# springmeyer/cov-tiles

Measured on AMD Instinct MI355X. Metric: GB/s raw COVT bytes decoded + Mvertices/s, z2–z14 tile batch, 1/2/4/8 GPU, higher is better.
Workload: dtype int32

## Files before the change

### cov-tiles_amd/csrc/covt_decode.hip

```cpp
#include <hip/hip_runtime.h>
#include <stdint.h>

#include "covt.h"
#include "covt_internal.h"
#include "covt_wave.h"
#include "covt_walk.h"

namespace covt {

constexpr int kWin = 1024;
constexpr int kFpfBlock = 256;
constexpr int kFpfPage = 65536;
constexpr int kFpfBcCap = 3 * kFpfPage / kFpfBlock + kFpfPage;

#ifndef COVT_LONG_STREAM
#define COVT_LONG_STREAM 16384
#endif
#ifndef COVT_LONG_PRIO
#define COVT_LONG_PRIO 2
#endif
#ifndef COVT_RLE_SHORT_SPAN
#define COVT_RLE_SHORT_SPAN 448
#endif
#ifndef COVT_CHUNK_PRIO
// ... 211 lines not shown
    const int32_t steps = (int32_t)wave_max((uint32_t)((nch + 15) >> 4));
    for (int32_t c0 = 0; c0 < 16 * steps; c0 += 16) {
        const int32_t ch = c0 + q;
        if (ch < nch) {
            const int32_t i = head + K * ch;
            int4 w;
            if (E == 8) {
                const int64_t v0 = val(i), v1 = val(i + 1);
                w = make_int4((int)v0, (int)(v0 >> 32), (int)v1, (int)(v1 >> 32));
            } else {
                w = make_int4((int)val(i), (int)val(i + 1), (int)val(i + 2), (int)val(i + 3));
            }
            st_out16((int32_t*)(arr + (int64_t)(o + i) * E), w);
        }
    }
}

template <int OP, int K>
__device__ __forceinline__ void sink_values(const uint32_t (&vin)[K], int64_t base, int32_t first, int32_t count,
                                            int nb, uint8_t* __restrict__ out, Carry& c) {
    const int l = lane_id();
    const bool full = first == 0 && count >= 64 * K;
    const int32_t s0 = l * K - first;
    const bool lfull = full || (s0 >= 0 && s0 + K <= count);
    const int64_t i0 = base + (int64_t)l * K;
    bool ok[K];
    uint32_t v[K];
#pragma unroll
    for (int k = 0; k < K; ++k) {
        ok[k] = full || (s0 + k >= 0 && s0 + k < count);
        v[k] = ok[k] ? vin[k] : 0u;
    }
    auto st32 = [&](const int32_t (&r)[K]) {
        int32_t* o = (int32_t*)out + i0;
        if (K == 4 && lfull) {
            st_out16(o, make_int4(r[0], r[K > 1 ? 1 : 0], r[K > 2 ? 2 : 0], r[K > 3 ? 3 : 0]));
        } else {
#pragma unroll
            for (int k = 0; k < K; ++k)
                if (ok[k]) st_out(o + k, r[k]);
        }
    };
    auto st64 = [&](const int64_t (&r)[K]) {
        int64_t* o = (int64_t*)out + i0;
#pragma unroll
        for (int k = 0; k < K; ++k)
            if (ok[k]) st_out(o + k, r[k]);
    };
    if constexpr (OP == COVT_OP_VARINT_I32 || OP == COVT_OP_VARINT_ZZ_I32) {
        int32_t r[K];
#pragma unroll
        for (int k = 0; k < K; ++k) r[k] = OP == COVT_OP_VARINT_I32 ? (int32_t)v[k] : zz32(v[k]);
        st32(r);
    } else if constexpr (OP == COVT_OP_VARINT_I32_AS_I64 || OP == COVT_OP_VARINT_ZZ_I32_AS_I64) {
        int64_t r[K];
#pragma unroll
        for (int k = 0; k < K; ++k) r[k] = OP == COVT_OP_VARINT_I32_AS_I64 ? (int64_t)(int32_t)v[k] : (int64_t)zz32(v[k]);
        st64(r);
    } else if constexpr (OP == COVT_OP_VARINT_ZZ_DELTA_I32 || OP == COVT_OP_FPF_ZZ_DELTA_I32 ||
                         OP == COVT_OP_VARINT_ZZ_DELTA_I64) {
        uint32_t sacc[K];
        uint32_t acc = 0;
#pragma unroll
        for (int k = 0; k < K; ++k) {
            acc += (uint32_t)zz32(v[k]);
            sacc[k] = acc;
        }
        const uint32_t inc = incl_scan(acc);
        const uint32_t pre = c.x + inc - acc;
        if constexpr (OP == COVT_OP_VARINT_ZZ_DELTA_I64) {
            int64_t r[K];
#pragma unroll
            for (int k = 0; k < K; ++k) r[k] = (int64_t)(int32_t)(pre + sacc[k]);
            st64(r);
        } else {
            int32_t r[K];
#pragma unroll
            for (int k = 0; k < K; ++k) r[k] = (int32_t)(pre + sacc[k]);
            st32(r);
        }
        c.x += lane_bcast(inc, 63);
    } else if constexpr (OP == COVT_OP_VARINT_ZZ_DELTA_XY || OP == COVT_OP_FPF_ZZ_DELTA_XY) {
        uint32_t sx[K], sy[K];
        uint32_t ax = 0, ay = 0;
        const uint32_t par0 = (uint32_t)(i0 & 1);
#pragma unroll
        for (int k = 0; k < K; ++k) {
            const uint32_t z = (uint32_t)zz32(v[k]);
            const bool isx = ((par0 + k) & 1u) == 0;
            ax += isx ? z : 0u;
            ay += isx ? 0u : z;
            sx[k] = ax;
            sy[k] = ay;
        }
        const uint32_t incx = incl_scan(ax), incy = incl_scan(ay);
        const uint32_t prex = c.x + incx - ax, prey = c.y + incy - ay;
        int32_t r[K];
#pragma unroll
        for (int k = 0; k < K; ++k) r[k] = (int32_t)((((par0 + k) & 1u) == 0) ? (prex + sx[k]) : (prey + sy[k]));
        st32(r);
        c.x += lane_bcast(incx, 63);
        c.y += lane_bcast(incy, 63);
    } else if constexpr (OP == COVT_OP_VARINT_DELTA_MORTON || OP == COVT_OP_FPF_DELTA_MORTON) {
        uint32_t sacc[K];
        uint32_t acc = 0;
#pragma unroll
        for (int k = 0; k < K; ++k) {
            acc += v[k];
            sacc[k] = acc;
        }
        const uint32_t inc = incl_scan(acc);
        const uint32_t pre = c.x + inc - acc;
        const int32_t half = morton_half(nb);
        int32_t* o = (int32_t*)out + 2 * i0;
        int32_t xy[2 * K];
#pragma unroll
        for (int k = 0; k < K; ++k) {
            uint32_t mx, my;
            morton_xy((int32_t)(pre + sacc[k]), nb, mx, my);
            xy[2 * k] = (int32_t)(mx - (uint32_t)half);
            xy[2 * k + 1] = (int32_t)(my - (uint32_t)half);
        }
        if (K == 4 && lfull) {
            st_out16(o, make_int4(xy[0], xy[1], xy[K > 1 ? 2 : 0], xy[K > 1 ? 3 : 0]));
            st_out16(o + 4, make_int4(xy[K > 2 ? 4 : 0], xy[K > 2 ? 5 : 0], xy[K > 3 ? 6 : 0], xy[K > 3 ? 7 : 0]));
        } else {
#pragma unroll
            for (int k = 0; k < K; ++k)
                if (ok[k]) st_out((int64_t*)(o + 2 * k), pack_xy(xy[2 * k], xy[2 * k + 1]));
        }
        c.x += lane_bcast(inc, 63);
    }
}

enum { MODE_RAW = 0, MODE_WORDREV = 1 };
enum { VAL_J4 = 0, VAL_VB = 1, VAL_U64 = 2, VAL_U64_STRICT = 3, VAL_NONE = 4 };

__device__ __forceinline__ uint32_t win_byte(const WaveSmem& sm, int32_t j) {
    return ((const uint8_t*)sm.u.v.win)[j];
}
__device__ __forceinline__ void win_bytes12(const WaveSmem& sm, int32_t j, uint32_t& x0, uint32_t& x1,
                                            uint32_t& x2) {
    const int32_t d = j >> 2;
    const uint32_t sh = (uint32_t)(j & 3);
    const uint32_t w0 = sm.u.v.win[d], w1 = sm.u.v.win[d + 1], w2 = sm.u.v.win[d + 2], w3 = sm.u.v.win[d + 3];
    x0 = __builtin_amdgcn_alignbyte(w1, w0, sh);
    x1 = __builtin_amdgcn_alignbyte(w2, w1, sh);
    x2 = __builtin_amdgcn_alignbyte(w3, w2, sh);
}

struct Win {
    int32_t woff;
    int32_t K;
    int32_t p0;
    bool valid, serial;
    uint4 d;
    uint32_t cpre, cmsk;
};

template <int MODE, int VAL>
__device__ void win_load(WaveSmem& sm, const uint8_t* sb, Win& w, int32_t p, int32_t end, const uint32_t* lsrc = nullptr,
                         int32_t lw0 = 0) {
    const int l = lane_id();
    uint4 d;
    int32_t woff;
    if (MODE == MODE_RAW) {
        const uintptr_t a = ((uintptr_t)(sb + p)) & ~(uintptr_t)15;
        woff = uni((int32_t)((intptr_t)a - (intptr_t)sb));
        d = woff + 16 * l < end ? ld128(a + 16 * (uintptr_t)l) : make_uint4(0, 0, 0, 0);
    } else {
        woff = p & ~15;
        const uint8_t* q = sb + woff + 16 * l;
        d = make_uint4(0, 0, 0, 0);
        if (woff + 16 * l < end) {
            if (lsrc) {
                const uint32_t* ws = lsrc + ((woff + 16 * l) >> 2) - lw0;
                d = make_uint4(ws[0], ws[1], ws[2], ws[3]);
            } else {
                d.x = ld_be32(q);
                d.y = ld_be32(q + 4);
                d.z = ld_be32(q + 8);
                d.w = ld_be32(q + 12);
            }
        }
        wave_sync();
    }
    ((uint4*)sm.u.v.win)[l] = d;
    if (VAL == VAL_NONE) {
        wave_sync();
        w.d = d;
        w.woff = woff;
        w.K = 0;
        w.p0 = p;
        w.valid = true;
        w.serial = false;
        return;
    }
    const int32_t q0 = woff + 16 * l;
    const uint32_t V = range16((VAL == VAL_J4 ? p : 0) - q0, end - q0);
    const uint32_t H = hibits16(d);
    uint32_t T = (VAL == VAL_VB) ? (V & H) : (V & ~H);
    bool serial = false;
    if (VAL == VAL_J4) {
        const uint32_t N = V & ~T;
        uint32_t prevN = (uint32_t)__shfl_up((int)N, 1, 64);
        if (l == 0) prevN = 0;
        const uint32_t ext = (N << 3) | ((prevN >> 13) & 7u);
        serial = __any((ext & (ext >> 1) & (ext >> 2) & (ext >> 3)) != 0);
    }
    int32_t K;
    if (!serial) {
        const uint32_t cnt = __popc(T);
        const uint32_t inc = incl_scan(cnt);
        uint32_t idx = inc - cnt;
        sm.cpre[l] = (uint16_t)idx;
        sm.cmask[l] = (uint16_t)T;
        w.cpre = idx;
        w.cmsk = T;
        while (T) {
            const int k = __ffs(T) - 1;
            T &= T - 1;
            sm.u.v.list[idx++] = (uint16_t)(16 * l + k);
        }
        K = (int32_t)lane_bcast(inc, 63);
    } else {
        wave_sync();
        if (l == 0) {
            const int32_t lim = (end < woff + kWin ? end : woff + kWin) - woff;
            int32_t j = p - woff, k = 0;
            while (j < lim) {
                int32_t len = 0;
                bool done = false;
                for (int b = 0; b < 4; ++b) {
                    if (j + b >= lim) break;
                    ++len;
                    if (b == 3 || (win_byte(sm, j + b) & 0x80u) == 0) { done = true; break; }
                }
                if (!done) break;
                sm.u.v.list[k++] = (uint16_t)(j + len - 1);
                j += len;
            }
            sm.misc[0] = k;
        }
        wave_sync();
        K = uni(sm.misc[0]);
    }
    wave_sync();
    w.d = d;
    w.woff = woff;
    w.K = K;
    w.p0 = p;
    w.valid = true;
    w.serial = serial || VAL == VAL_J4;
}

__device__ __forceinline__ int32_t win_rank(const WaveSmem& sm, const Win& w, int32_t q) {
    const int32_t j = q - w.woff;
    if (j <= 0) return 0;
    if (j >= kWin) return w.K;
    const int32_t c = j >> 4;
    return (int32_t)uniu((uint32_t)sm.cpre[c] + __popc((uint32_t)sm.cmask[c] & ((1u << (j & 15)) - 1u)));
}

template <int VAL>
__device__ __forceinline__ void win_value(const WaveSmem& sm, int32_t sj, int32_t ej, uint32_t& lo, uint32_t& hi,
                                          bool& lerr) {
    const int32_t len = ej - sj + 1;
    uint32_t x0, x1, x2;
    win_bytes12(sm, sj, x0, x1, x2);
    lo = 0;
    hi = 0;
    if (VAL == VAL_J4) {
        lo = pext7(x0 & bytemask(len));
    } else if (VAL == VAL_VB) {
        if (len <= 5) {
            lo = pext7(x0 & bytemask(len));
            if (len == 5) lo += (x1 & 0x7fu) << 28;
        } else {
            uint32_t vv = 0;
            for (int b = 0; b < len; ++b) vv += (win_byte(sm, sj + b) & 0x7fu) << ((7 * b) & 31);
            lo = vv;
        }
    } else {
        uint64_t rv;
        if (len <= 10) {
            const uint32_t m0 = x0 & bytemask(len), m1 = x1 & bytemask(len - 4), m2 = x2 & bytemask(len - 8);
            rv = (uint64_t)pext7(m0) | ((uint64_t)pext7(m1) << 28) | ((uint64_t)(m2 & 0x7fu) << 56) |
                 ((uint64_t)((m2 >> 8) & 0x7fu) << 63);
        } else {
            rv = 0;
            for (int b = 0; b < len; ++b) rv |= (uint64_t)(win_byte(sm, sj + b) & 0x7fu) << ((7 * b) & 63);
            lerr = true;
        }
        lo = (uint32_t)rv;
        hi = (uint32_t)(rv >> 32);
    }
}

#ifndef COVT_VARINT_LINES
#define COVT_VARINT_LINES 1
#endif
template <int MODE, int VAL, int K = 1, class Emit>
__device__ int32_t varint_take(WaveSmem& sm, const uint8_t* sb, Win& w, int32_t& pos, int32_t end, int32_t want,
                               bool until_end, int32_t& err, Emit&& emit, int32_t out0 = 0,
                               int32_t* first_bad = nullptr, int32_t line = 0, const uint32_t* lsrc = nullptr,
                               int32_t lw0 = 0) {
    const int l = lane_id();
    int32_t got = 0;
    while (until_end ? (pos < end) : (got < want)) {
        if (!w.valid || pos < w.woff || pos >= w.woff + kWin || (w.serial && pos != w.p0)) {
            win_load<MODE, VAL>(sm, sb, w, pos, end, lsrc, lw0);
            lsrc = nullptr;
        }
        const int32_t r = w.serial ? 0 : win_rank(sm, w, pos);
        const int32_t have = w.K - r;
        if (have <= 0) {
            const int32_t aligned = (MODE == MODE_RAW) ? (int32_t)(((uintptr_t)(sb + pos) & ~(uintptr_t)15) -
                                                                   (uintptr_t)sb)
                                                       : (pos & ~15);
            if (w.woff != aligned) {
                win_load<MODE, VAL>(sm, sb, w, pos, end);
                continue;
            }
            if (until_end) break;
            err = (w.woff + kWin >= end) ? COVT_ERR_TRUNCATED : COVT_ERR_BAD_HEADER;
            break;
        }
        int32_t take = have;
        if (until_end) {
            if (got + have > want) { err = COVT_ERR_COUNT_MISMATCH; take = want - got; }
        } else if (take > want - got) {
            take = want - got;
        }
        if (take <= 0) break;
        if (COVT_VARINT_LINES && MODE == MODE_RAW && line && !until_end && got + take < want) {
            const int32_t cut = (out0 + got + take) & (line - 1);
            if (cut < take) {
                take -= cut;
            } else {
                const int32_t aligned = (int32_t)(((uintptr_t)(sb + pos) & ~(uintptr_t)15) - (uintptr_t)sb);
                if (w.woff != aligned) {
                    win_load<MODE, VAL>(sm, sb, w, pos, end);
                    continue;
                }
            }
        }
        bool lerr = false;
        int32_t fb = INT32_MAX;
        const int32_t s0 = pos - w.woff;
        const int32_t lead = (K > 1) ? ((out0 + got) & (K - 1)) : 0;
        for (int32_t g = -lead; g < take; g += 64 * K) {
            uint32_t lo[K], hi[K];
#pragma unroll
            for (int k = 0; k < K; ++k) {
                int32_t vi = g + K * l + k;
                vi = vi < 0 ? 0 : (vi < take ? vi : take - 1);
                const int32_t li = r + vi - 1;
                const int32_t pv = (int32_t)sm.u.v.list[li < 0 ? 0 : li] + 1;
                const int32_t sj = vi == 0 ? s0 : pv;
                if constexpr (VAL == VAL_J4) {
                    const int32_t dq = sj >> 2;
                    const uint32_t x = __builtin_amdgcn_alignbyte(sm.u.v.win[dq + 1], sm.u.v.win[dq], (uint32_t)sj & 3u);
                    const uint32_t u = ~x & 0x80808080u;
                    lo[k] = pext7(x & (u ^ (u - 1u)));
                    hi[k] = 0;
                } else {
                    bool lk = false;
                    win_value<VAL>(sm, sj, sm.u.v.list[r + vi], lo[k], hi[k], lk);
                    if (VAL == VAL_U64_STRICT && first_bad && lk) fb = min(fb, got + vi);
                    lerr = lerr || lk;
                }
            }
            const int32_t first = g < 0 ? -g : 0;
            const int32_t cnt = (take - g < 64 * K ? take - g : 64 * K) - first;
            emit(lo, hi, got + g, first, cnt);
        }
        if (VAL == VAL_U64_STRICT && __any(lerr) && !err) {
            err = COVT_ERR_BAD_HEADER;
            if (first_bad) *first_bad = (int32_t)~wave_max(~(uint32_t)fb);
        }
        pos = w.woff + (int32_t)uniu(sm.u.v.list[r + take - 1]) + 1;
        if (w.serial) { w.p0 = pos; w.valid = false; }
        got += take;
        if (err) break;
    }
    return got;
}

struct Ctx {
    WaveSmem* sm;
    const uint8_t* sb;
    uint8_t* out;
    int32_t avail, n, nb, op, byte_length;
    int32_t err, consumed;
#ifdef COVT_TIMING
    uint64_t ph_last;
    uint32_t ph[kPhases];
#endif
};
#ifdef COVT_TIMING
#define COVT_PHASE(c, k)                                          \
    do {                                                          \
        const uint64_t t_ = __builtin_amdgcn_s_memtime();         \
        (c).ph[k] += (uint32_t)(t_ - (c).ph_last);                \
        (c).ph_last = t_;                                         \
    } while (0)
#else
#define COVT_PHASE(c, k) \
    do {                 \
    } while (0)
#endif

template <int VAL>
__device__ __forceinline__ uint32_t rd_byte(Ctx& c, Win& w, int32_t q, int32_t need = 1) {
    if (!w.valid || q < w.woff || (q + need > w.woff + kWin && w.woff + kWin < c.avail))
        win_load<MODE_RAW, VAL>(*c.sm, c.sb, w, q, c.avail);
    return uniu(win_byte(*c.sm, q - w.woff));
}

template <int OP>
__device__ __forceinline__ void sink_u64(const uint32_t (&lo)[4], const uint32_t (&hi)[4], int64_t base, int32_t first,
                                         int32_t count, int64_t* o, uint64_t& acc) {
    const int32_t s0 = 4 * lane_id() - first;
    int64_t* p = o + base + 4 * lane_id();
    uint64_t v[4];
#pragma unroll
    for (int k = 0; k < 4; ++k) {
        const bool ok = s0 + k >= 0 && s0 + k < count;
        v[k] = ok ? (((uint64_t)hi[k] << 32) | lo[k]) : 0ull;
        if constexpr (OP != COVT_OP_VARINT_U64) v[k] = (uint64_t)zz64(v[k]);
    }
    if constexpr (OP == COVT_OP_VARINT_ZZ_DELTA_S64) {
        uint64_t sacc = 0;
#pragma unroll
        for (int k = 0; k < 4; ++k) {
            sacc += v[k];
            v[k] = sacc;
        }
        const uint64_t inc = incl_scan64(sacc);
        const uint64_t pre = acc + inc - sacc;
#pragma unroll
        for (int k = 0; k < 4; ++k) v[k] += pre;
        acc += lane_bcast64(inc, 63);
    }
    if (s0 >= 0 && s0 + 4 <= count) {
        st_out16((int32_t*)p, make_int4((int)v[0], (int)(v[0] >> 32), (int)v[1], (int)(v[1] >> 32)));
        st_out16((int32_t*)(p + 2), make_int4((int)v[2], (int)(v[2] >> 32), (int)v[3], (int)(v[3] >> 32)));
    } else {
#pragma unroll
        for (int k = 0; k < 4; ++k)
            if (s0 + k >= 0 && s0 + k < count) st_out(p + k, (int64_t)v[k]);
    }
}

template <int OP>
__device__ __forceinline__ void run_varint_stream(Ctx& c) {
    constexpr int32_t kLine = (OP == COVT_OP_VARINT_I32_AS_I64 || OP == COVT_OP_VARINT_ZZ_I32_AS_I64 ||
                               OP == COVT_OP_VARINT_ZZ_DELTA_I64 || OP == COVT_OP_VARINT_DELTA_MORTON) ? 16 : 32;
    int32_t pos = 0;
    Carry cr{0, 0};
    Win w;
    w.valid = false;
    auto sink4 = [&](const uint32_t (&lo)[4], const uint32_t (&hi)[4], int32_t base, int32_t first, int32_t count) {
        sink_values<OP, 4>(lo, base, first, count, c.nb, c.out, cr);
    };
    if constexpr (OP == COVT_OP_VARINT_U64 || OP == COVT_OP_VARINT_ZZ_S64 || OP == COVT_OP_VARINT_ZZ_DELTA_S64) {
        uint64_t acc = 0;
        varint_take<MODE_RAW, VAL_U64_STRICT, 4>(
            *c.sm, c.sb, w, pos, c.avail, c.n, false, c.err,
            [&](const uint32_t (&lo)[4], const uint32_t (&hi)[4], int32_t base, int32_t first, int32_t count) {
                sink_u64<OP>(lo, hi, base, first, count, (int64_t*)c.out, acc);
            },
            0, nullptr, 16);
    } else {
        if ((OP == COVT_OP_VARINT_ZZ_DELTA_XY) && (c.n & 1)) {
            varint_take<MODE_RAW, VAL_J4, 4>(*c.sm, c.sb, w, pos, c.avail, c.n - 1, false, c.err, sink4, 0, nullptr,
                                             kLine);
            if (!c.err) c.err = COVT_ERR_COUNT_MISMATCH;
        } else {
            varint_take<MODE_RAW, VAL_J4, 4>(*c.sm, c.sb, w, pos, c.avail, c.n, false, c.err, sink4, 0, nullptr, kLine);
        }
    }
    c.consumed = pos;
}

__device__ __forceinline__ int32_t rank_rel(const WaveSmem& sm, int32_t j, int32_t K) {
    if (j >= kWin) return K;
    const int32_t c = j >> 4;
    return (int32_t)sm.cpre[c] + __popc((uint32_t)sm.cmask[c] & ((1u << (j & 15)) - 1u));
}
__device__ __forceinline__ uint64_t win_vulong(const WaveSmem& sm, int32_t sj, int32_t ej) {
    const int32_t len = ej - sj + 1;
    if (len <= 10) {
        uint32_t x0, x1, x2;
        win_bytes12(sm, sj, x0, x1, x2);
        const uint32_t m0 = x0 & bytemask(len), m1 = x1 & bytemask(len - 4), m2 = x2 & bytemask(len - 8);
        return (uint64_t)pext7(m0) | ((uint64_t)pext7(m1) << 28) | ((uint64_t)(m2 & 0x7fu) << 56) |
               ((uint64_t)((m2 >> 8) & 0x7fu) << 63);
    }
    uint64_t r = 0;
    for (int b = 0; b < len; ++b) r |= (uint64_t)(win_byte(sm, sj + b) & 0x7fu) << ((7 * b) & 63);
    return r;
}
__device__ __forceinline__ uint32_t win_vulong_lo32(const WaveSmem& sm, int32_t sj, int32_t ej) {
    const int32_t len = ej - sj + 1;
    if (len > 10) return (uint32_t)win_vulong(sm, sj, ej);
    const int32_t d = sj >> 2;
    const uint32_t sh = (uint32_t)(sj & 3);
    const uint32_t w0 = sm.u.v.win[d], w1 = sm.u.v.win[d + 1], w2 = sm.u.v.win[d + 2];
    const uint32_t x0 = __builtin_amdgcn_alignbyte(w1, w0, sh), x1 = __builtin_amdgcn_alignbyte(w2, w1, sh);
    return pext7(x0 & bytemask(len)) | (len >= 5 ? (x1 & 0x7fu) << 28 : 0u);
}

__device__ __forceinline__ void run_rle_int(Ctx& c, int32_t o0 = 0) {
    WaveSmem& sm = *c.sm;
    const int l = lane_id();
    const bool is_signed = c.op == COVT_OP_RLE_S64;
    const bool to_i32 = c.op == COVT_OP_RLE_I32;
    Win w;
    w.valid = false;
    int32_t pos = 0, done = o0;
    auto store = [&](int64_t i, uint64_t raw) {
        const int64_t v = is_signed ? zz64(raw) : (int64_t)raw;
        if (to_i32) st_out((int32_t*)c.out + i, (int32_t)v);
        else st_out((int64_t*)c.out + i, v);
    };
    while (done < c.n && !c.err) {
        if (pos >= c.avail) { c.err = COVT_ERR_TRUNCATED; break; }
        COVT_PHASE(c, 7);
        win_load<MODE_RAW, VAL_U64>(sm, c.sb, w, pos, c.avail);
        COVT_PHASE(c, 0);
        const int32_t woff = w.woff, K = w.K;
        const int32_t jlo = pos - woff;
        const uint32_t nb = (uint32_t)(uintptr_t)(lds_cu16*)&sm.u.v.next[0];
        const uint32_t sent = nb + 2u * (uint32_t)kWin;
// ... 1264 lines not shown
        if (!c.err && p < nw32) {
            int32_t vpos = (int32_t)(4 * p);
            const int32_t base = L;
            Win w;
            w.valid = false;
            const bool tail_in = L > 0 && ((vpos & ~15) >> 2) >= mw0 && nw32 - mw0 <= 255;
            const int32_t got = varint_take<MODE_WORDREV, VAL_VB>(
                sm, c.sb, w, vpos, 4 * nw32, c.n - L, true, c.err,
                [&](const uint32_t (&lo)[1], const uint32_t (&hi)[1], int32_t vb, int32_t, int32_t count) {
                    sink_values<OP, 1>(lo, (int64_t)base + vb, 0, count, c.nb, c.out, cr);
                },
                0, nullptr, 0, tail_in ? sm.u.f.cbuf : nullptr, (int32_t)mw0);
            decoded = L + got;
        }
    }
    if (!c.err) {
        for (int32_t b = decoded; b < c.n; b += 64) {
            uint32_t vv[1] = {0};
            sink_values<OP, 1>(vv, b, 0, c.n - b < 64 ? c.n - b : 64, c.nb, c.out, cr);
        }
        if (OP == COVT_OP_FPF_ZZ_DELTA_XY && (c.n & 1)) c.err = COVT_ERR_COUNT_MISMATCH;
    }
    COVT_PHASE(c, 7);
    c.consumed = c.byte_length;
}

template <int OP>
__device__ __forceinline__ void fpf_add_carry(uint8_t* out, int32_t v0, int32_t v1, Carry cr) {
    const uint32_t cx = cr.x, cy = OP == COVT_OP_FPF_ZZ_DELTA_XY ? cr.y : cr.x;
    if ((cx | cy) == 0u) return;
    __builtin_amdgcn_s_waitcnt(0x0f70);
    int32_t* o = (int32_t*)out;
    typedef __attribute__((address_space(1))) i32x4 g_i4;
    const int32_t nq = (v1 - v0) >> 2;
    const int32_t last = v0 + 4 * (nq > 0 ? nq - 1 : 0);
    constexpr int kDeep = 8;
    for (int32_t q0 = 0; q0 < nq; q0 += 64 * kDeep) {
        i32x4 v[kDeep];
#pragma unroll
        for (int k = 0; k < kDeep; ++k) v[k] = *(const g_i4*)(o + min(v0 + 4 * (q0 + 64 * k + lane_id()), last));
#pragma unroll
        for (int k = 0; k < kDeep; ++k) {
            const int32_t q = q0 + 64 * k + lane_id();
            if (q < nq)
                st_out16(o + v0 + 4 * q, make_int4((int32_t)((uint32_t)v[k].x + cx), (int32_t)((uint32_t)v[k].y + cy),
                                                   (int32_t)((uint32_t)v[k].z + cx), (int32_t)((uint32_t)v[k].w + cy)));
        }
    }
    const int32_t i = v0 + 4 * nq + lane_id();
    if (i < v1) o[i] = (int32_t)((uint32_t)o[i] + (((i - v0) & 1) ? cy : cx));
}

constexpr int kSplitSlots = COVT_SPLIT_SLOTS;
struct Agg {
    int32_t cnt;
    uint32_t sx, sy;
};
__device__ __forceinline__ Agg agg_cat(const Agg& a, const Agg& b, bool xy) {
    if (a.cnt < 0) return a;
    if (b.cnt < 0) return Agg{b.cnt, b.sx, (uint32_t)a.cnt + b.sy};
    const bool sw = xy && (a.cnt & 1);
    return Agg{a.cnt + b.cnt, a.sx + (sw ? b.sy : b.sx), a.sy + (sw ? b.sx : b.sy)};
}
typedef __attribute__((address_space(1))) uint64_t g_u64;
__device__ __forceinline__ void rec_publish(covt_stream_result* rec, const Agg& a, uint32_t tag) {
    if (lane_id() == 0) {
        g_u64* g = (g_u64*)rec;
        const uint64_t t = (uint64_t)tag << 32;
        __hip_atomic_store(g, t | (uint32_t)a.cnt, __ATOMIC_RELAXED, __HIP_MEMORY_SCOPE_AGENT);
        __hip_atomic_store(g + 1, t | a.sx, __ATOMIC_RELAXED, __HIP_MEMORY_SCOPE_AGENT);
        __hip_atomic_store(g + 2, t | a.sy, __ATOMIC_RELAXED, __HIP_MEMORY_SCOPE_AGENT);
    }
}
__device__ __forceinline__ bool rec_try(covt_stream_result* rec, uint32_t tag, Agg& a) {
    g_u64* g = (g_u64*)rec;
    const uint64_t x0 = __hip_atomic_load(g, __ATOMIC_RELAXED, __HIP_MEMORY_SCOPE_AGENT);
    const uint64_t x1 = __hip_atomic_load(g + 1, __ATOMIC_RELAXED, __HIP_MEMORY_SCOPE_AGENT);
    const uint64_t x2 = __hip_atomic_load(g + 2, __ATOMIC_RELAXED, __HIP_MEMORY_SCOPE_AGENT);
    const bool ok = (uint32_t)(x0 >> 32) == tag && (uint32_t)(x1 >> 32) == tag && (uint32_t)(x2 >> 32) == tag;
    a = Agg{(int32_t)(uint32_t)x0, (uint32_t)x1, (uint32_t)x2};
    return uniu(ok ? 1u : 0u) != 0u;
}
constexpr int kRecAgg = 1, kRecIncl = 4, kRecTicket = 7;
static_assert(kSplitSlots == 8, "split record layout");
constexpr uint32_t kSpinLimit = 1u << 22;
__device__ Agg lookback(covt_stream_result* res, int64_t t, int32_t chunk, bool xy, int32_t& err) {
    Agg acc{0, 0u, 0u};
    int64_t k = t - 1;
    uint32_t spins = 0;
    for (int32_t left = chunk; left > 0;) {
        covt_stream_result* r = res + kSplitSlots * k;
        Agg a;
        if (rec_try(r + kRecIncl, 2u, a)) {
            acc = agg_cat(a, acc, xy);
            break;
        }
        if (rec_try(r + kRecAgg, 1u, a)) {
            acc = agg_cat(a, acc, xy);
            --k;
            --left;
            continue;
        }
        if (++spins > kSpinLimit) { err = COVT_ERR_DEVICE; break; }
        __builtin_amdgcn_s_sleep(2);
    }
    return acc;
}

template <int OP>
__device__ __forceinline__ void run_varint_chunk(Ctx& c, int32_t s, int32_t e, int32_t chunk, covt_stream_result* res, int64_t t) {
    constexpr bool kU64 = OP == COVT_OP_VARINT_U64 || OP == COVT_OP_VARINT_ZZ_S64;
    constexpr int kVal = kU64 ? VAL_U64_STRICT : VAL_J4;
    constexpr bool kXY = OP == COVT_OP_VARINT_ZZ_DELTA_XY;
    constexpr bool kZZ = OP == COVT_OP_VARINT_ZZ_I32 || OP == COVT_OP_VARINT_ZZ_DELTA_I32 || kXY ||
                         OP == COVT_OP_VARINT_ZZ_I32_AS_I64 || OP == COVT_OP_VARINT_ZZ_DELTA_I64;
    constexpr bool kSum = OP == COVT_OP_VARINT_ZZ_DELTA_I32 || kXY || OP == COVT_OP_VARINT_DELTA_MORTON ||
                          OP == COVT_OP_VARINT_ZZ_DELTA_I64;
    const int l = lane_id();
    int32_t p = 0;
    if (chunk > 0) {
        const uintptr_t lo = (uintptr_t)c.sb & ~(uintptr_t)15;
        int32_t hi = s, last = -1;
        while (hi > 0) {
            uintptr_t w0 = ((uintptr_t)(c.sb + hi) & ~(uintptr_t)15);
            w0 = w0 >= lo + 1008 ? w0 - 1008 : lo;
            const uint4 d = ld128(w0 + 16 * (uintptr_t)l);
            const int32_t q0 = (int32_t)((intptr_t)(w0 + 16 * (uintptr_t)l) - (intptr_t)c.sb);
            const uint32_t T = ~hibits16(d) & 0xffffu & range16(-q0, hi - q0);
            const uint32_t best = T ? (uint32_t)(q0 + 31 - __builtin_clz(T)) + 1u : 0u;
            const uint32_t m = wave_max(best);
            if (m) { last = (int32_t)m - 1; break; }
            hi = (int32_t)((intptr_t)w0 - (intptr_t)c.sb);
        }
        p = last + 1;
        while (!kU64 && p < s) {
            const uint32_t x = uniu(ld_le32(c.sb + p));
            const uint32_t u = ~x & 0x80808080u;
            const int32_t len = u ? (__builtin_ctz(u) >> 3) + 1 : 4;
            if (p + len - 1 >= s) break;
            p += len;
        }
    }
    Win w;
    int32_t err = 0, ferr = 0, cnt = 0, take = 0, pos = p, bad = -1;
    Agg excl{0, 0u, 0u};
#pragma nounroll
    for (int pass = 0; pass < 2; ++pass) {
        uint32_t ax = 0, ay = 0;
        Carry cr{excl.sx, excl.sy};
        uint64_t acc = 0;
        const int32_t g0 = excl.cnt;
        w.valid = false;
        pos = p;
        const int32_t got = varint_take<MODE_RAW, kVal, 4>(
            *c.sm, c.sb, w, pos, e, pass == 0 ? INT32_MAX : take, pass == 0, err,
            [&](const uint32_t (&lo)[4], const uint32_t (&hi)[4], int32_t base, int32_t first, int32_t count) {
                if (pass == 1) {
                    if constexpr (kU64) sink_u64<OP>(lo, hi, (int64_t)g0 + base, first, count, (int64_t*)c.out, acc);
                    else sink_values<OP, 4>(lo, (int64_t)g0 + base, first, count, c.nb, c.out, cr);
                } else if (kSum) {
                    const int32_t s0 = 4 * l - first;
#pragma unroll
                    for (int k = 0; k < 4; ++k) {
                        const bool ok = s0 + k >= 0 && s0 + k < count;
                        const uint32_t z = ok ? (kZZ ? (uint32_t)zz32(lo[k]) : lo[k]) : 0u;
                        const bool odd = kXY && (((uint32_t)(base + 4 * l + k)) & 1u);
                        ax += odd ? 0u : z;
                        ay += odd ? z : 0u;
                    }
                }
            },
            pass == 0 ? 0 : g0, &bad);
        if (pass == 1) break;
        cnt = got;
        if (kU64 && err) {
            cnt = bad;
        } else if (kU64 && pos < e) {
            const int32_t aligned = (int32_t)(((uintptr_t)(c.sb + pos) & ~(uintptr_t)15) - (uintptr_t)c.sb);
            if (aligned + kWin < e) {
                err = COVT_ERR_BAD_HEADER;
                bad = cnt;
            }
        }
        Agg mine{cnt, 0u, 0u};
        if (err) {
            mine = Agg{INT32_MIN, (uint32_t)err, (uint32_t)cnt};
        } else if (kSum) {
            mine.sx = lane_bcast(incl_scan(ax), 63);
            mine.sy = kXY ? lane_bcast(incl_scan(ay), 63) : 0u;
        }
        covt_stream_result* rec = res + kSplitSlots * t;
        int32_t lerr = 0;
        if (chunk == 0) {
            rec_publish(rec + kRecIncl, mine, 2u);
        } else {
            rec_publish(rec + kRecAgg, mine, 1u);
            excl = lookback(res, t, chunk, kXY, lerr);
            rec_publish(rec + kRecIncl, lerr ? Agg{INT32_MIN, (uint32_t)lerr, 0u} : agg_cat(excl, mine, kXY), 2u);
        }
        if (lerr) {
            err = lerr;
            bad = 0;
            excl = Agg{0, 0u, 0u};
            break;
        }
        if (excl.cnt < 0) return;
        if (err && excl.cnt + bad < c.n) ferr = err;
        err = 0;
        take = min(cnt, c.n - excl.cnt);
        pos = p;
        if (take <= 0) break;
    }
    if (ferr) err = ferr;
    covt_stream_result* r0 = res + kSplitSlots * (t - chunk);
    const bool has_last = !err && excl.cnt < c.n && excl.cnt + cnt >= c.n;
    const bool short_end = !err && e >= c.byte_length && excl.cnt + cnt < c.n;
    if (l == 0 && (has_last || short_end || err)) {
        covt_stream_result r;
        r.status = err ? err : (has_last ? COVT_OK : COVT_ERR_TRUNCATED);
        r.consumed = pos;
        *r0 = r;
    }
}

template <int OP>
__device__ __forceinline__ void run_fastpfor_chunk(Ctx& c, int32_t v0, int32_t v1, int32_t chunk, covt_stream_result* res,
                                   int64_t t, const covt_stream_desc* __restrict__ cd) {
    constexpr bool kXY = OP == COVT_OP_FPF_ZZ_DELTA_XY;
    Carry carry{0u, 0u};
    int32_t err = 0;
    FpfSkip skip;
    {
        auto slot = [&](int i) -> const int32_t* {
            return (const int32_t*)((const uint8_t*)(cd + 2 + i / 7) + covt_fpf_state_byte(i % 7));
        };
        if (uni(*slot(0)) == 1) {
            const int l = lane_id();
            skip.done = uni(*slot(1));
            skip.cur0 = uni(*slot(2));
            skip.pk = uni(*slot(3));
            skip.xc = l <= 32 ? *slot(4 + l) : 0;
        }
    }
    constexpr bool kOnce = OP != COVT_OP_FPF_DELTA_MORTON;
    static_assert(OP == COVT_OP_FPF_ZZ_DELTA_I32 || OP == COVT_OP_FPF_ZZ_DELTA_XY || OP == COVT_OP_FPF_DELTA_MORTON,
                  "split FastPFOR op without a carry rule");
    static_assert(!kOnce || OP == COVT_OP_FPF_ZZ_DELTA_I32 || OP == COVT_OP_FPF_ZZ_DELTA_XY,
                  "in-place carry only for the linear int32 ops");
#pragma nounroll
    for (int pass = 0; pass < 2; ++pass) {
        Carry sums{0u, 0u};
        c.err = 0;
        run_fastpfor<OP>(c, v0, v1, carry, pass == 0 && !kOnce, &sums, &skip, kOnce ? &sums : nullptr);
        if (pass == 1) {
            err = c.err;
            break;
        }
        const int32_t own_err = c.err;
        const Agg mine = own_err ? Agg{INT32_MIN, (uint32_t)own_err, 0u} : Agg{v1 - v0, sums.x, sums.y};
        covt_stream_result* rec = res + kSplitSlots * t;
        Agg excl{0, 0u, 0u};
        if (chunk == 0) {
            rec_publish(rec + kRecIncl, mine, 2u);
        } else {
            rec_publish(rec + kRecAgg, mine, 1u);
            excl = lookback(res, t, chunk, kXY, err);
            rec_publish(rec + kRecIncl, err ? Agg{INT32_MIN, (uint32_t)err, 0u} : agg_cat(excl, mine, kXY), 2u);
        }
        if (!err && excl.cnt < 0) err = (int32_t)excl.sx;
        if (!err) err = own_err;
        if (err) break;
        carry = Carry{excl.sx, excl.sy};
        if (kOnce) {
            fpf_add_carry<OP>(c.out, v0, v1 < c.n ? v1 : c.n, carry);
            break;
        }
    }
    if (lane_id() == 0 && (v1 >= c.n || err)) {
        covt_stream_result r;
        r.status = err;
        r.consumed = c.byte_length;
        res[kSplitSlots * (t - chunk)] = r;
    }
}

__device__ __forceinline__ void run_rle_chunk(Ctx& c, const covt_stream_desc* __restrict__ cd, int32_t chunk, covt_stream_result* res,
                              int64_t t) {
    const int32_t s = (int32_t)cd[1].in_off, e = (int32_t)cd[1].out_off;
    const int32_t v0 = (int32_t)cd[2].in_off, nv = (int32_t)cd[2].out_off;
    c.sb += s;
    c.avail = c.byte_length = e - s;
    c.n = v0 + nv;
    if (c.op == COVT_OP_BYTE_RLE_U8 || c.op == COVT_OP_BYTE_RLE_RAW) run_rle_byte(c, v0, true);
    else run_rle_int(c, v0);
    if (lane_id() == 0) {
        covt_stream_result* r0 = res + kSplitSlots * (t - chunk);
        if (c.err) atomicMin(&r0->status, c.err);
        if (chunk == 0) r0->consumed = (int32_t)cd[3].in_off;
    }
}

constexpr int kSplitVarint = 0, kSplitFpf = 1, kSplitRle = 2;
template <int K>
__device__ __forceinline__ int64_t decode_split_chunk(WaveSmem* sm, const uint8_t* __restrict__ in, const covt_stream_desc* __restrict__ descs,
                                      int64_t n_chunks, uint8_t* __restrict__ out, covt_stream_result* __restrict__ res) {
    constexpr bool FPF = K == kSplitFpf;
    uint32_t* ctr = (uint32_t*)(res + kRecTicket);
// ... 645 lines not shown
```

### cov-tiles_amd/csrc/covt_wave.h

```cpp
#ifndef COVT_WAVE_H
#define COVT_WAVE_H

#include <hip/hip_runtime.h>
#include <stdint.h>

namespace covt {

__device__ __forceinline__ int lane_id() { return __lane_id(); }
__device__ __forceinline__ int32_t uni(int32_t x) { return __builtin_amdgcn_readfirstlane(x); }
__device__ __forceinline__ uint32_t uniu(uint32_t x) { return (uint32_t)__builtin_amdgcn_readfirstlane((int)x); }
__device__ __forceinline__ int64_t uni64(int64_t x) {
    const uint32_t lo = uniu((uint32_t)x), hi = uniu((uint32_t)((uint64_t)x >> 32));
    return (int64_t)(((uint64_t)hi << 32) | lo);
}
__device__ __forceinline__ uint32_t lane_bcast(uint32_t x, int src) {
    return (uint32_t)__builtin_amdgcn_readlane((int)x, src);
}
__device__ __forceinline__ void wave_sync() {
    __builtin_amdgcn_fence(__ATOMIC_SEQ_CST, "wavefront");
    __builtin_amdgcn_wave_barrier();
}
__device__ __forceinline__ uint32_t incl_scan(uint32_t x) {
    x += (uint32_t)__builtin_amdgcn_update_dpp(0, (int)x, 0x111, 0xf, 0xf, false);
    x += (uint32_t)__builtin_amdgcn_update_dpp(0, (int)x, 0x112, 0xf, 0xf, false);
    x += (uint32_t)__builtin_amdgcn_update_dpp(0, (int)x, 0x114, 0xf, 0xf, false);
    x += (uint32_t)__builtin_amdgcn_update_dpp(0, (int)x, 0x118, 0xf, 0xf, false);
    x += (uint32_t)__builtin_amdgcn_update_dpp(0, (int)x, 0x142, 0xa, 0xf, false);
    x += (uint32_t)__builtin_amdgcn_update_dpp(0, (int)x, 0x143, 0xc, 0xf, false);
    return x;
}

__device__ __forceinline__ uint32_t add_sat(uint32_t a, uint32_t b) { return __builtin_elementwise_add_sat(a, b); }
__device__ __forceinline__ uint32_t incl_scan_sat(uint32_t x) {
    x = add_sat(x, (uint32_t)__builtin_amdgcn_update_dpp(0, (int)x, 0x111, 0xf, 0xf, false));
    x = add_sat(x, (uint32_t)__builtin_amdgcn_update_dpp(0, (int)x, 0x112, 0xf, 0xf, false));
    x = add_sat(x, (uint32_t)__builtin_amdgcn_update_dpp(0, (int)x, 0x114, 0xf, 0xf, false));
    x = add_sat(x, (uint32_t)__builtin_amdgcn_update_dpp(0, (int)x, 0x118, 0xf, 0xf, false));
    x = add_sat(x, (uint32_t)__builtin_amdgcn_update_dpp(0, (int)x, 0x142, 0xa, 0xf, false));
    x = add_sat(x, (uint32_t)__builtin_amdgcn_update_dpp(0, (int)x, 0x143, 0xc, 0xf, false));
    return x;
}

__device__ __forceinline__ uint64_t incl_scan64(uint64_t x) {
    uint32_t lo = (uint32_t)x, hi = (uint32_t)(x >> 32);
#define COVT_SCAN64_STEP(ctrl, rmask)                                                             \
    {                                                                                             \
        const uint32_t l2 = (uint32_t)__builtin_amdgcn_update_dpp(0, (int)lo, ctrl, rmask, 0xf, false); \
        const uint32_t h2 = (uint32_t)__builtin_amdgcn_update_dpp(0, (int)hi, ctrl, rmask, 0xf, false); \
        const uint32_t s = lo + l2;                                                               \
        hi = hi + h2 + (s < lo ? 1u : 0u);                                                        \
        lo = s;                                                                                   \
    }
    COVT_SCAN64_STEP(0x111, 0xf)
    COVT_SCAN64_STEP(0x112, 0xf)
    COVT_SCAN64_STEP(0x114, 0xf)
    COVT_SCAN64_STEP(0x118, 0xf)
    COVT_SCAN64_STEP(0x142, 0xa)
    COVT_SCAN64_STEP(0x143, 0xc)
#undef COVT_SCAN64_STEP
    return ((uint64_t)hi << 32) | lo;
}
__device__ __forceinline__ uint64_t lane_bcast64(uint64_t x, int src) {
    return ((uint64_t)lane_bcast((uint32_t)(x >> 32), src) << 32) | lane_bcast((uint32_t)x, src);
}

__device__ __forceinline__ uint32_t incl_max_scan(uint32_t x) {
    x = max(x, (uint32_t)__builtin_amdgcn_update_dpp(0, (int)x, 0x111, 0xf, 0xf, false));
    x = max(x, (uint32_t)__builtin_amdgcn_update_dpp(0, (int)x, 0x112, 0xf, 0xf, false));
    x = max(x, (uint32_t)__builtin_amdgcn_update_dpp(0, (int)x, 0x114, 0xf, 0xf, false));
    x = max(x, (uint32_t)__builtin_amdgcn_update_dpp(0, (int)x, 0x118, 0xf, 0xf, false));
    x = max(x, (uint32_t)__builtin_amdgcn_update_dpp(0, (int)x, 0x142, 0xa, 0xf, false));
    x = max(x, (uint32_t)__builtin_amdgcn_update_dpp(0, (int)x, 0x143, 0xc, 0xf, false));
    return x;
}

__device__ __forceinline__ uint32_t wave_max(uint32_t x) {
    x = max(x, (uint32_t)__builtin_amdgcn_update_dpp(0, (int)x, 0x111, 0xf, 0xf, false));
    x = max(x, (uint32_t)__builtin_amdgcn_update_dpp(0, (int)x, 0x112, 0xf, 0xf, false));
    x = max(x, (uint32_t)__builtin_amdgcn_update_dpp(0, (int)x, 0x114, 0xf, 0xf, false));
    x = max(x, (uint32_t)__builtin_amdgcn_update_dpp(0, (int)x, 0x118, 0xf, 0xf, false));
    x = max(x, (uint32_t)__builtin_amdgcn_update_dpp(0, (int)x, 0x142, 0xa, 0xf, false));
    x = max(x, (uint32_t)__builtin_amdgcn_update_dpp(0, (int)x, 0x143, 0xc, 0xf, false));
    return lane_bcast(x, 63);
}

__device__ __forceinline__ uint64_t wave_or64(uint64_t v) {
    uint32_t lo = (uint32_t)v, hi = (uint32_t)(v >> 32);
#define COVT_OR64_STEP(ctrl, rmask)                                                    \
    lo |= (uint32_t)__builtin_amdgcn_update_dpp(0, (int)lo, ctrl, rmask, 0xf, false); \
    hi |= (uint32_t)__builtin_amdgcn_update_dpp(0, (int)hi, ctrl, rmask, 0xf, false);
    COVT_OR64_STEP(0x111, 0xf)
    COVT_OR64_STEP(0x112, 0xf)
    COVT_OR64_STEP(0x114, 0xf)
    COVT_OR64_STEP(0x118, 0xf)
    COVT_OR64_STEP(0x142, 0xa)
    COVT_OR64_STEP(0x143, 0xc)
#undef COVT_OR64_STEP
    return ((uint64_t)lane_bcast(hi, 63) << 32) | lane_bcast(lo, 63);
}

__device__ __forceinline__ uint32_t lane_next(uint32_t x, uint32_t tail = 0) {
    return (uint32_t)__builtin_amdgcn_update_dpp((int)tail, (int)x, 0x130, 0xf, 0xf, false);
}
__device__ __forceinline__ int32_t bits_below(uint64_t m) {
    return (int32_t)__builtin_amdgcn_mbcnt_hi((uint32_t)(m >> 32), __builtin_amdgcn_mbcnt_lo((uint32_t)m, 0u));
}
__device__ __forceinline__ int32_t lane_get(int32_t x, int32_t src) {
    return __builtin_amdgcn_ds_bpermute(src << 2, x);
}

}

#endif
```

Measured before the change: 675.1.

## Add dedicated compacting decoder for Java-capped 4-byte varints with lookahead loads

Moves the VAL_J4 (max-4-byte varint) path out of the generic window/rank machinery into a specialised reader. It finds terminator bytes with a dot-product bitmask, then scatters each value's 4 raw bytes directly into LDS slots using branchless address selection. Values are then decoded in 256-wide vector groups, and the next 16-byte-per-lane window is prefetched while the current one is processed. The per-window serial/p0 state is removed from the generic path. This is meant to cut the LDS list indirection and load latency on the hot zigzag stream, at the cost of inline asm complexity and a separate serial fallback path.

```diff
diff --git a/cov-tiles_amd/csrc/covt_decode.hip b/cov-tiles_amd/csrc/covt_decode.hip
--- a/cov-tiles_amd/csrc/covt_decode.hip
+++ b/cov-tiles_amd/csrc/covt_decode.hip
@@ -387,8 +387,7 @@
 struct Win {
     int32_t woff;
     int32_t K;
-    int32_t p0;
-    bool valid, serial;
+    bool valid;
     uint4 d;
     uint32_t cpre, cmsk;
 };
@@ -426,67 +425,30 @@
         w.d = d;
         w.woff = woff;
         w.K = 0;
-        w.p0 = p;
         w.valid = true;
-        w.serial = false;
         return;
     }
     const int32_t q0 = woff + 16 * l;
-    const uint32_t V = range16((VAL == VAL_J4 ? p : 0) - q0, end - q0);
+    const uint32_t V = range16(-q0, end - q0);
     const uint32_t H = hibits16(d);
     uint32_t T = (VAL == VAL_VB) ? (V & H) : (V & ~H);
-    bool serial = false;
-    if (VAL == VAL_J4) {
-        const uint32_t N = V & ~T;
-        uint32_t prevN = (uint32_t)__shfl_up((int)N, 1, 64);
-        if (l == 0) prevN = 0;
-        const uint32_t ext = (N << 3) | ((prevN >> 13) & 7u);
-        serial = __any((ext & (ext >> 1) & (ext >> 2) & (ext >> 3)) != 0);
-    }
-    int32_t K;
-    if (!serial) {
-        const uint32_t cnt = __popc(T);
-        const uint32_t inc = incl_scan(cnt);
-        uint32_t idx = inc - cnt;
-        sm.cpre[l] = (uint16_t)idx;
-        sm.cmask[l] = (uint16_t)T;
-        w.cpre = idx;
-        w.cmsk = T;
-        while (T) {
-            const int k = __ffs(T) - 1;
-            T &= T - 1;
-            sm.u.v.list[idx++] = (uint16_t)(16 * l + k);
-        }
-        K = (int32_t)lane_bcast(inc, 63);
-    } else {
-        wave_sync();
-        if (l == 0) {
-            const int32_t lim = (end < woff + kWin ? end : woff + kWin) - woff;
-            int32_t j = p - woff, k = 0;
-            while (j < lim) {
-                int32_t len = 0;
-                bool done = false;
-                for (int b = 0; b < 4; ++b) {
-                    if (j + b >= lim) break;
-                    ++len;
-                    if (b == 3 || (win_byte(sm, j + b) & 0x80u) == 0) { done = true; break; }
-                }
-                if (!done) break;
-                sm.u.v.list[k++] = (uint16_t)(j + len - 1);
-                j += len;
-            }
-            sm.misc[0] = k;
-        }
-        wave_sync();
-        K = uni(sm.misc[0]);
+    const uint32_t cnt = __popc(T);
+    const uint32_t inc = incl_scan(cnt);
+    uint32_t idx = inc - cnt;
+    sm.cpre[l] = (uint16_t)idx;
+    sm.cmask[l] = (uint16_t)T;
+    w.cpre = idx;
+    w.cmsk = T;
+    while (T) {
+        const int k = __ffs(T) - 1;
+        T &= T - 1;
+        sm.u.v.list[idx++] = (uint16_t)(16 * l + k);
     }
     wave_sync();
     w.d = d;
     w.woff = woff;
-    w.K = K;
-    w.p0 = p;
+    w.K = (int32_t)lane_bcast(inc, 63);
     w.valid = true;
-    w.serial = serial || VAL == VAL_J4;
 }
 
 __device__ __forceinline__ int32_t win_rank(const WaveSmem& sm, const Win& w, int32_t q) {
@@ -505,9 +467,7 @@
     win_bytes12(sm, sj, x0, x1, x2);
     lo = 0;
     hi = 0;
-    if (VAL == VAL_J4) {
-        lo = pext7(x0 & bytemask(len));
-    } else if (VAL == VAL_VB) {
+    if (VAL == VAL_VB) {
         if (len <= 5) {
             lo = pext7(x0 & bytemask(len));
             if (len == 5) lo += (x1 & 0x7fu) << 28;
@@ -535,19 +495,178 @@
 #ifndef COVT_VARINT_LINES
 #define COVT_VARINT_LINES 1
 #endif
-template <int MODE, int VAL, int K = 1, class Emit>
+
+constexpr int kJ4Slots = (kWin / 4 + 4) + kWin / 2;
+constexpr int kJ4Cap = 768;
+constexpr int kJ4SerBase = kWin / 4 + 4;
+constexpr int kJ4SerEnds = kJ4SerBase + 256;
+constexpr int kJ4SerCap = 252;
+static_assert(kJ4Cap + 3 + 1 <= kJ4Slots && kJ4Cap % 32 == 0, "slot buffer");
+static_assert(kJ4SerEnds + 256 <= kJ4Slots && kJ4SerCap + 3 < 256, "serial slot buffer");
+typedef __attribute__((address_space(3))) uint32_t lds_u32;
+__device__ __forceinline__ uint32_t hibits16_dot(uint4 d) {
+    const uint32_t lo = ((d.x >> 7) & 0x01010101u) | ((d.y >> 3) & 0x10101010u);
+    const uint32_t hi = ((d.z >> 7) & 0x01010101u) | ((d.w >> 3) & 0x10101010u);
+    return __builtin_amdgcn_udot4(lo, 0x08040201u, 0u, false) | (__builtin_amdgcn_udot4(hi, 0x08040201u, 0u, false) << 8);
+}
+
+template <bool AHEAD, class Emit>
+__device__ int32_t varint_take_j4(WaveSmem& sm, const uint8_t* sb, int32_t& pos, int32_t end, int32_t want,
+                                  bool until_end, int32_t& err, Emit&& emit, int32_t out0, int32_t line) {
+    const int l = lane_id();
+    uint32_t* const slots = sm.u.v.win;
+    int32_t got = 0;
+    auto load_at = [&](int32_t p) -> uint4 {
+        const uintptr_t a = ((uintptr_t)(sb + p)) & ~(uintptr_t)15;
+        const int32_t q = uni((int32_t)((intptr_t)a - (intptr_t)sb)) + 16 * l;
+        return q < end ? ld128(a + 16 * (uintptr_t)l) : make_uint4(0, 0, 0, 0);
+    };
+    uint4 dn = make_uint4(0, 0, 0, 0);
+    bool ahead = false;
+    while (until_end ? (pos < end) : (got < want)) {
+        const uintptr_t a = ((uintptr_t)(sb + pos)) & ~(uintptr_t)15;
+        const int32_t woff = uni((int32_t)((intptr_t)a - (intptr_t)sb));
+        const int32_t q0 = woff + 16 * l;
+        const uint4 d = ahead ? dn : load_at(pos);
+        const uint32_t V = range16(pos - q0, end - q0);
+        const uint32_t T = V & ~hibits16_dot(d);
+        const uint32_t N = V & ~T;
+        const uint32_t ext = (N << 3) | ((lane_prev(N) >> 13) & 7u);
+        const bool serial = __any((ext & (ext >> 1) & (ext >> 2) & (ext >> 3)) != 0);
+        const int32_t lead = (out0 + got) & 3;
+        const uint32_t cnt = __popc(T);
+        uint32_t inc = 0;
+        int32_t K;
+        wave_sync();
+        if (!serial) {
+            inc = incl_scan(cnt);
+            K = (int32_t)lane_bcast(inc, 63);
+        } else {
+            ((uint4*)sm.u.v.win)[l] = d;
+            wave_sync();
+            if (l == 0) {
+                const int32_t lim = (end < woff + kWin ? end : woff + kWin) - woff;
+                int32_t j = pos - woff, k = 0;
+                while (j < lim && k < kJ4SerCap) {
+                    int32_t len = 0;
+                    bool done = false;
+                    for (int b = 0; b < 4; ++b) {
+                        if (j + b >= lim) break;
+                        ++len;
+                        if (b == 3 || (win_byte(sm, j + b) & 0x80u) == 0) { done = true; break; }
+                    }
+                    if (!done) break;
+                    const int32_t dq = j >> 2;
+                    slots[kJ4SerBase + lead + k] =
+                        __builtin_amdgcn_alignbyte(sm.u.v.win[dq + 1], sm.u.v.win[dq], (uint32_t)j & 3u);
+                    slots[kJ4SerEnds + k] = (uint32_t)(j + len - 1);
+                    ++k;
+                    j += len;
+                }
+                sm.misc[0] = k;
+            }
+            wave_sync();
+            K = uni(sm.misc[0]);
+        }
+        if (K <= 0) {
+            if (until_end) break;
+            err = (woff + kWin >= end) ? COVT_ERR_TRUNCATED : COVT_ERR_BAD_HEADER;
+            break;
+        }
+        int32_t take = K;
+        if (until_end) {
+            if (got + K > want) { err = COVT_ERR_COUNT_MISMATCH; take = want - got; }
+        } else if (take > want - got) {
+            take = want - got;
+        }
+        if (take <= 0) break;
+        if (take > kJ4Cap) take = kJ4Cap;
+        if (COVT_VARINT_LINES && line && !until_end && got + take < want) {
+            const int32_t cut = (out0 + got + take) & (line - 1);
+            if (cut < take) take -= cut;
+        }
+        int32_t npos;
+        auto load_ahead = [&]() {
+            ahead = AHEAD && !err && (until_end ? npos < end : got + take < want);
+            if (ahead) dn = load_at(npos);
+        };
+        if (!serial) {
+            const int32_t lp = (int32_t)__builtin_ctzll(__ballot(inc > (uint32_t)(take - 1)));
+            const uint32_t tl = lane_bcast(T, lp);
+            const uint32_t nth = (uint32_t)(take - 1) - lane_bcast(inc - cnt, lp);
+            const uint32_t jb = (uint32_t)l & 15u;
+            const int32_t b = (int32_t)__builtin_ctzll(
+                __ballot(((tl >> jb) & 1u) != 0 && (uint32_t)__popc(tl & ((1u << jb) - 1u)) == nth));
+            npos = woff + 16 * lp + b + 1;
+            load_ahead();
+            const uint32_t tm = l < lp ? T : (l == lp ? T & ((2u << b) - 1u) : 0u);
+            const uint32_t S = (tm << 1) | lane_prev(tm >> 15) | (l == 0 ? 1u << (pos - woff) : 0u);
+            const uint32_t dw[5] = {d.x, d.y, d.z, d.w, lane_next(d.x)};
+            uint32_t sa = (uint32_t)(uintptr_t)(lds_u32*)(slots + lead + (int32_t)(inc - cnt) - (l == 0 && pos > woff ? 1 : 0));
+            const uint32_t da = (uint32_t)(uintptr_t)(lds_u32*)((uint32_t*)sm.cpre + l);
+            int32_t m;
+            asm("v_bfe_i32 %0, %1, 0, 1" : "=v"(m) : "v"(S));
+#define COVT_J4_POS(j)                                                                                          \
+    {                                                                                                           \
+        const uint32_t x =                                                                                      \
+            ((j) & 3) ? __builtin_amdgcn_alignbyte(dw[(j) / 4 + 1], dw[(j) / 4], (uint32_t)((j) & 3)) : dw[(j) / 4]; \
+        uint32_t wa;                                                                                            \
+        asm("v_bfi_b32 %0, %1, %2, %3" : "=v"(wa) : "v"(m), "v"(sa), "v"(da));                                  \
+        *(lds_u32*)(uintptr_t)wa = x;                                                                           \
+        if ((j) < 15) {                            \
+            asm("v_bfe_i32 %0, %1, %2, 1" : "=v"(m) : "v"(S), "n"((j) + 1));                                    \
+            asm("v_mad_i32_i24 %0, %1, -4, %2" : "=v"(sa) : "v"(m), "v"(sa));                                   \
+        }                                                                                                       \
+    }
+            COVT_J4_POS(0) COVT_J4_POS(1) COVT_J4_POS(2) COVT_J4_POS(3) COVT_J4_POS(4) COVT_J4_POS(5)
+            COVT_J4_POS(6) COVT_J4_POS(7) COVT_J4_POS(8) COVT_J4_POS(9) COVT_J4_POS(10) COVT_J4_POS(11)
+            COVT_J4_POS(12) COVT_J4_POS(13) COVT_J4_POS(14) COVT_J4_POS(15)
+#undef COVT_J4_POS
+        } else {
+            npos = woff + (int32_t)uniu(slots[kJ4SerEnds + take - 1]) + 1;
+            load_ahead();
+        }
+        wave_sync();
+        const int32_t sbase = serial ? kJ4SerBase : 0, smax = serial ? 252 : kJ4Slots - 4;
+        for (int32_t g = -lead; g < take; g += 256) {
+            const int32_t s = g + lead + 4 * l;
+            const uint4 r = *(const uint4*)(slots + sbase + (s < smax ? s : smax));
+            const uint32_t x[4] = {r.x, r.y, r.z, r.w};
+            uint32_t lo[4], hi[4];
+#pragma unroll
+            for (int k = 0; k < 4; ++k) {
+                const uint32_t u = ~x[k] & 0x80808080u;
+                lo[k] = pext7(x[k] & (u ^ (u - 1u)));
+                hi[k] = 0;
+            }
+            const int32_t first = g < 0 ? -g : 0;
+            const int32_t n = (take - g < 256 ? take - g : 256) - first;
+            emit(lo, hi, got + g, first, n);
+        }
+        pos = npos;
+        got += take;
+        if (err) break;
+    }
+    return got;
+}
+
+template <int MODE, int VAL, int K = 1, bool AHEAD = true, class Emit>
 __device__ int32_t varint_take(WaveSmem& sm, const uint8_t* sb, Win& w, int32_t& pos, int32_t end, int32_t want,
                                bool until_end, int32_t& err, Emit&& emit, int32_t out0 = 0,
                                int32_t* first_bad = nullptr, int32_t line = 0, const uint32_t* lsrc = nullptr,
                                int32_t lw0 = 0) {
+    if constexpr (VAL == VAL_J4) {
+        static_assert(MODE == MODE_RAW && K == 4, "the compacting path is the only Java-capped reader");
+        return varint_take_j4<AHEAD>(sm, sb, pos, end, want, until_end, err, emit, out0, line);
+    }
     const int l = lane_id();
     int32_t got = 0;
     while (until_end ? (pos < end) : (got < want)) {
-        if (!w.valid || pos < w.woff || pos >= w.woff + kWin || (w.serial && pos != w.p0)) {
+        if (!w.valid || pos < w.woff || pos >= w.woff + kWin) {
             win_load<MODE, VAL>(sm, sb, w, pos, end, lsrc, lw0);
             lsrc = nullptr;
         }
-        const int32_t r = w.serial ? 0 : win_rank(sm, w, pos);
+        const int32_t r = win_rank(sm, w, pos);
         const int32_t have = w.K - r;
         if (have <= 0) {
             const int32_t aligned = (MODE == MODE_RAW) ? (int32_t)(((uintptr_t)(sb + pos) & ~(uintptr_t)15) -
@@ -593,18 +712,10 @@
                 const int32_t li = r + vi - 1;
                 const int32_t pv = (int32_t)sm.u.v.list[li < 0 ? 0 : li] + 1;
                 const int32_t sj = vi == 0 ? s0 : pv;
-                if constexpr (VAL == VAL_J4) {
-                    const int32_t dq = sj >> 2;
-                    const uint32_t x = __builtin_amdgcn_alignbyte(sm.u.v.win[dq + 1], sm.u.v.win[dq], (uint32_t)sj & 3u);
-                    const uint32_t u = ~x & 0x80808080u;
-                    lo[k] = pext7(x & (u ^ (u - 1u)));
-                    hi[k] = 0;
-                } else {
-                    bool lk = false;
-                    win_value<VAL>(sm, sj, sm.u.v.list[r + vi], lo[k], hi[k], lk);
-                    if (VAL == VAL_U64_STRICT && first_bad && lk) fb = min(fb, got + vi);
-                    lerr = lerr || lk;
-                }
+                bool lk = false;
+                win_value<VAL>(sm, sj, sm.u.v.list[r + vi], lo[k], hi[k], lk);
+                if (VAL == VAL_U64_STRICT && first_bad && lk) fb = min(fb, got + vi);
+                lerr = lerr || lk;
             }
             const int32_t first = g < 0 ? -g : 0;
             const int32_t cnt = (take - g < 64 * K ? take - g : 64 * K) - first;
@@ -615,7 +726,6 @@
             if (first_bad) *first_bad = (int32_t)~wave_max(~(uint32_t)fb);
         }
         pos = w.woff + (int32_t)uniu(sm.u.v.list[r + take - 1]) + 1;
-        if (w.serial) { w.p0 = pos; w.valid = false; }
         got += take;
         if (err) break;
     }
@@ -2186,7 +2296,7 @@
         const int32_t g0 = excl.cnt;
         w.valid = false;
         pos = p;
-        const int32_t got = varint_take<MODE_RAW, kVal, 4>(
+        const int32_t got = varint_take<MODE_RAW, kVal, 4, false>(
             *c.sm, c.sb, w, pos, e, pass == 0 ? INT32_MAX : take, pass == 0, err,
             [&](const uint32_t (&lo)[4], const uint32_t (&hi)[4], int32_t base, int32_t first, int32_t count) {
                 if (pass == 1) {
diff --git a/cov-tiles_amd/csrc/covt_wave.h b/cov-tiles_amd/csrc/covt_wave.h
--- a/cov-tiles_amd/csrc/covt_wave.h
+++ b/cov-tiles_amd/csrc/covt_wave.h
@@ -102,6 +102,9 @@
 __device__ __forceinline__ uint32_t lane_next(uint32_t x, uint32_t tail = 0) {
     return (uint32_t)__builtin_amdgcn_update_dpp((int)tail, (int)x, 0x130, 0xf, 0xf, false);
 }
+__device__ __forceinline__ uint32_t lane_prev(uint32_t x, uint32_t head = 0) {
+    return (uint32_t)__builtin_amdgcn_update_dpp((int)head, (int)x, 0x138, 0xf, 0xf, false);
+}
 __device__ __forceinline__ int32_t bits_below(uint64_t m) {
     return (int32_t)__builtin_amdgcn_mbcnt_hi((uint32_t)(m >> 32), __builtin_amdgcn_mbcnt_lo((uint32_t)m, 0u));
 }
```

After: 617.7. -8.5%, worse.
